# amplab/keystone

Measured on NVIDIA H100. Metric: block-LS fit samples/sec (N=1M, D=64K, k=1K), higher is better.
Workload: dtype f16x2

## Files before the change

### keystone_b200/csrc/engine.cu

```cuda
#include "engine.h"

#include <cuda_fp16.h>
#include <dlfcn.h>
#include <stdlib.h>
#include <math.h>
#include <string.h>

#include <chrono>
#include <functional>
#include <mutex>
#include <sstream>

namespace ks {

template <class F>
static void load_sym(void* lib, const char* name, F& out, const char* libname) {
  void* s = dlsym(lib, name);
  if (!s) throw KsError{KS_ERR_SOLVER, std::string("symbol ") + name + " missing from " + libname};
  out = reinterpret_cast<F>(s);
}
static void* open_first(const std::vector<const char*>& names) {
  for (const char* n : names) {
    void* h = dlopen(n, RTLD_NOW | RTLD_GLOBAL);
    if (h) return h;
// ... 493 lines not shown
  float* slab = static_cast<float*>(slab_v);
  if (src.F) {
    if (!round_out || out16 || x2) throw KsError{KS_ERR_INVALID, "unrounded / fp16 slabs only for generated features"};
    launch_center_round(src.F->d + row_begin * src.F->ld, src.F->ld, static_cast<int>(c0), shift, slab, colsum, lds, rows,
                        static_cast<int>(cols), st);
    c.launches += 1;
    return;
  }
  KmLaunch k;
  int64_t kdepth = src.d_in;
  if (x2) {
    if (!src.proj_x2 || out16 || round_out) throw KsError{KS_ERR_INVALID, "split-operand slab requested without split operands"};
    kdepth = 3 * src.d_in;
    tmap16_or_throw(&k.tmA, static_cast<const uint16_t*>(src.x3.p) + row_begin * src.ldx3, rows, kdepth, src.ldx3, 64, 128, TMAP_SW128);
    tmap16_or_throw(&k.tmB, static_cast<const uint16_t*>(src.w3.p) + c0 * src.ldw3, cols, kdepth, src.ldw3, 64, 128, TMAP_SW128);
    k.f16 = 1;
    k.p.acc_scale_ptr = src.pscale.as<float>();
  } else if (out16 && src.proj16) {
    tmap16_or_throw(&k.tmA, static_cast<const uint16_t*>(src.xop16.p) + row_begin * src.X->ld, rows, src.d_in, src.X->ld, 64, 128,
                    TMAP_SW128);
    tmap16_or_throw(&k.tmB, static_cast<const uint16_t*>(src.w16.p) + c0 * src.ldw, cols, src.d_in, src.ldw, 64, 128, TMAP_SW128);
    k.f16 = 1;
    k.p.acc_scale_ptr = src.pscale.as<float>();
  } else {
    tmap_or_throw(&k.tmA, src.xop.as<float>() + row_begin * src.X->ld, rows, src.d_in, src.X->ld, 128);
    tmap_or_throw(&k.tmB, src.Wall + c0 * src.ldw, cols, src.d_in, src.ldw, 128);
  }
  if (slab_lo && !x2) throw KsError{KS_ERR_INVALID, "a lo plane needs the split operands"};
  if (slab_lo) {
    tmap16_or_throw(&k.tmOut, slab_v, rows, cols, lds, 32, 32, TMAP_NONE);
    tmap16_or_throw(&k.tmOut2, slab_lo, rows, cols, lds, 32, 32, TMAP_NONE);
    k.out16 = 2;
  } else {
    if (out16) tmap16_or_throw(&k.tmOut, slab_v, rows, cols, lds, 32, 32, TMAP_NONE);
    else tmap_or_throw(&k.tmOut, slab, rows, cols, lds, 32);
    k.out16 = out16 ? 1 : 0;
  }
  k.p.vec0 = src.ball + c0;
  k.p.vec1 = shift;
  k.p.colsum = colsum;
  k.p.colsumsq = colsumsq;
  k.p.M = static_cast<int>(rows);
  k.p.N = static_cast<int>(cols);
  k.p.K = static_cast<int>(kdepth);
  k.p.flags = (round_out ? 0 : KM_FLAG_NO_ROUND) | (src.kind == 1 ? KM_FLAG_RECT : 0);
  k.p.rect_floor = src.rect_floor;
  k.epi = EPI_COS;
  k.num_sms = (st == c.st2) ? std::max(1, c.num_sms - c.reserve_sms) : c.num_sms;
  if (c.dyn_tiles) k.p.tile_counter = c.next_tile_counter(st);
  KS_CUDA(launch_kmajor(k, st));
  c.launches += 1;
}

const GramTile* gram_tiles(Ctx& c, int b, int kcols, bool with_g, bool with_c, int* num_tiles) {
  std::vector<int> key = {b, kcols, with_g ? 1 : 0, with_c ? 1 : 0};
  auto it = c.tile_cache.find(key);
  std::vector<GramTile> t;
  const int tm = 128, tn = 128;
  const int mb = (b + tm - 1) / tm;
  if (with_g) {
    const int nbk = (b + tn - 1) / tn;
    for (int i = 0; i < mb; ++i)
      for (int j = 0; j < nbk; ++j)
        if ((j + 1) * tn - 1 >= i * tm) t.push_back(GramTile{i, j, 0, 0});
  }
  if (with_c) {
    const int nck = (kcols + tn - 1) / tn;
    for (int i = 0; i < mb; ++i)
      for (int j = 0; j < nck; ++j) t.push_back(GramTile{i, j, 1, 0});
  }
  *num_tiles = static_cast<int>(t.size());
  if (it != c.tile_cache.end()) return it->second->as<GramTile>();
  auto buf = std::make_unique<DevBuf>();
  buf->alloc(sizeof(GramTile) * std::max<size_t>(t.size(), 1));
  KS_CUDA(cudaMemcpyAsync(buf->p, t.data(), sizeof(GramTile) * t.size(), cudaMemcpyHostToDevice, c.st));
  KS_CUDA(cudaStreamSynchronize(c.st));
  const GramTile* p = buf->as<GramTile>();
  c.tile_cache[key] = std::move(buf);
  return p;
}

void launch_gram_block(Ctx& c, const void* slab, int64_t lds, int64_t rows, int b, const void* R, int64_t ldr, int kcols,
                       float* G, int ldg, float* C, int ldc, bool with_g, bool with_c, cudaStream_t st, bool f16,
                       int64_t chunk_rows, const void* slab_lo, const void* R_lo) {
  if (rows <= 0 || b <= 0 || (!with_g && !with_c)) return;
  if (!st) st = c.st;
  const bool split = slab_lo != nullptr;
  if (split && (!f16 || (with_c && !R_lo))) throw KsError{KS_ERR_INVALID, "split Gram operands must be fp16 pairs"};
  GramLaunch g;
  int nt = 0;
  g.f16 = f16 ? 1 : 0;
  g.split = split ? 1 : 0;
  g.tiles = gram_tiles(c, b, kcols, with_g, with_c, &nt);
  g.num_tiles = nt;
  const int stage_rows = split ? 32 : f16 ? 64 : kGramStageRows;
  if (f16) {
    tmap16_or_throw(&g.tmA, slab, rows, b, lds, 64, stage_rows, TMAP_SW128);
    g.tmB0 = g.tmA;
    if (with_c) tmap16_or_throw(&g.tmB1, R, rows, kcols, ldr, 64, stage_rows, TMAP_SW128);
    else g.tmB1 = g.tmA;
    if (split) {
      tmap16_or_throw(&g.tmAlo, slab_lo, rows, b, lds, 64, stage_rows, TMAP_SW128);
      g.tmB0lo = g.tmAlo;
      if (with_c) tmap16_or_throw(&g.tmB1lo, R_lo, rows, kcols, ldr, 64, stage_rows, TMAP_SW128);
      else g.tmB1lo = g.tmAlo;
    }
  } else {
    tmap_or_throw(&g.tmA, static_cast<const float*>(slab), rows, b, lds, kGramStageRows);
    g.tmB0 = g.tmA;
    if (with_c) tmap_or_throw(&g.tmB1, static_cast<const float*>(R), rows, kcols, ldr, kGramStageRows);
    else g.tmB1 = g.tmA;
  }
  g.rows = static_cast<int>(rows);
  int64_t chunk = chunk_rows > 0 ? chunk_rows : c.gram_chunk_rows;
  if (chunk <= 0) chunk = !f16 ? 4096 : rows >= 400000 ? 16384 : rows >= 200000 ? 8192 : 4096;
  chunk = std::max<int64_t>(stage_rows, chunk / stage_rows * stage_rows);
  g.chunk_rows = static_cast<int>(chunk);
  if (with_g) tmap_or_throw(&g.tmOut0, G, b, b, ldg, 32);
  if (with_c) tmap_or_throw(&g.tmOut1, C, b, kcols, ldc, 32);
  if (!with_g) g.tmOut0 = g.tmOut1;
  if (!with_c) g.tmOut1 = g.tmOut0;
  g.n_valid0 = b;
  g.n_valid1 = kcols;
  KS_CUDA(launch_gram(g, st));
  c.launches += 1;
}

void launch_update(Ctx& c, const void* slab, int64_t lds, int64_t rows, int b, const void* bop, int64_t ldb, int k,
                   float* out, int64_t ldo, const float* cbias, int epi, bool reduce, cudaStream_t st, bool f16,
                   const float* acc_scale_ptr, const void* slab_lo, const void* bop_lo) {
  if (rows <= 0 || k <= 0 || b <= 0) return;
  if (!st) st = c.st;
  const bool split = slab_lo != nullptr;
  if (split && (!f16 || !bop_lo || epi != EPI_UPDATE)) throw KsError{KS_ERR_INVALID, "split update operands must be fp16 pairs"};
  KmLaunch u;
  u.f16 = f16 ? 1 : 0;
  u.split = split ? 1 : 0;
  u.p.acc_scale_ptr = acc_scale_ptr;
  if (split) {
    tmap16_or_throw(&u.tmA, slab, rows, b, lds, 32, 128, TMAP_SW64);
    tmap16_or_throw(&u.tmAlo, slab_lo, rows, b, lds, 32, 128, TMAP_SW64);
    tmap16_or_throw(&u.tmB, bop, k, b, ldb, 32, 128, TMAP_SW64);
    tmap16_or_throw(&u.tmBlo, bop_lo, k, b, ldb, 32, 128, TMAP_SW64);
  } else if (f16) {
    tmap16_or_throw(&u.tmA, slab, rows, b, lds, 64, 128, TMAP_SW128);
    tmap16_or_throw(&u.tmB, bop, k, b, ldb, 64, 128, TMAP_SW128);
  } else {
// ... 2152 lines not shown
```

### keystone_b200/csrc/engine.h

```cpp
#pragma once
#include <cuda_runtime.h>
#include <cusolverDn.h>
#include <nccl.h>
#include <stdint.h>

#include <map>
#include <memory>
#include <string>
#include <unordered_map>
#include <vector>

#include "../../include/keystone_b200.h"
#include "kernels.h"

namespace ks {

struct KsError {
  int code;
  std::string msg;
};

#define KS_CUDA(call)                                                                                   \
  do {                                                                                                  \
    cudaError_t e__ = (call);                                                                           \
// ... 238 lines not shown
  int64_t add(std::unique_ptr<Matrix> m);
  int64_t add(std::unique_ptr<Model> m);
  cudaEvent_t get_event();
  void span_begin(int phase, cudaStream_t s = nullptr);
  void span_end(cudaStream_t s = nullptr);
  void collect_spans(double out_ms[PH_COUNT]);
  void allreduce_f32(float* p, size_t n, bool prep = false);
  void allreduce_f64(double* p, size_t n, bool prep = false);
  void allreduce_on(void* p, size_t n, bool f64, ncclComm_t cm, cudaStream_t s);
  DevBuf tile_counters;
  int tile_counter_next = 0;
  int dyn_tiles = 1;
  int* next_tile_counter(cudaStream_t s);
  std::vector<cudaEvent_t> fit_events;
  void allreduce_max_u32(unsigned* p, size_t n);
  void ensure_solver();
  void potrf(double* H, int n, int info_slot, cudaStream_t s);
  void potrs(const double* H, int n, double* B, int nrhs, int info_slot, cudaStream_t s);
  void check_infos(int used_slots);
  void check_async(const char* what);
};

struct FeatMap {
  float* Wall = nullptr;
  float* Wfull = nullptr;
  int kind = 0;
  float rect_floor = 0.f;
  float* ball = nullptr;
  int64_t ldw = 0, d_in = 0;
  int64_t D = 0;
};
struct FeatSrc : FeatMap {
  Matrix* F = nullptr;
  Matrix* X = nullptr;
  DevBuf xop;
  DevBuf xop16, w16, pscale;
  bool proj16 = false;
  DevBuf x3, w3;
  int64_t ldx3 = 0, ldw3 = 0;
  bool proj_x2 = false;
  DevBuf wcat, wcat_full, bcat;
  int64_t n_rows = 0;
  DevBuf zeros;
};
void make_feat_src(Ctx& c, int64_t features, int64_t x_in, const int64_t* rfs, int32_t n_rfs, FeatSrc& out,
                   int precision = 0);
void prepare_generated_operands(Ctx& c, FeatSrc& out, int precision);
void derive_feat_src(Ctx& c, const FeatSrc& src, Matrix* X, FeatSrc& out, int precision);
void produce_slab(Ctx& c, FeatSrc& src, int64_t c0, int64_t cols, const float* shift, void* slab, int64_t lds,
                  int64_t row_begin, int64_t rows, bool round_out = true, float* colsum = nullptr, cudaStream_t st = nullptr,
                  bool out16 = false, bool x2 = false,
                  void* slab_lo = nullptr,
                  double* colsumsq = nullptr);
const GramTile* gram_tiles(Ctx& c, int b, int kcols, bool with_g, bool with_c, int* num_tiles);
void launch_gram_block(Ctx& c, const void* slab, int64_t lds, int64_t rows, int b, const void* R, int64_t ldr, int kcols,
                       float* G, int ldg, float* C, int ldc, bool with_g, bool with_c, cudaStream_t st = nullptr,
                       bool f16 = false, int64_t chunk_rows = 0,
                       const void* slab_lo = nullptr, const void* R_lo = nullptr);
void launch_update(Ctx& c, const void* slab, int64_t lds, int64_t rows, int b, const void* bop, int64_t ldb, int k,
                   float* out, int64_t ldo, const float* cbias, int epi, bool reduce, cudaStream_t st = nullptr,
                   bool f16 = false, const float* acc_scale_ptr = nullptr,
                   const void* slab_lo = nullptr, const void* bop_lo = nullptr);

int64_t fit_bwls(Ctx& c, FeatSrc& src, Matrix& Y, int bs, int num_iter, double lam, double w, int64_t nf_opt,
                 int precision = KS_PRECISION_TF32);
void launch_set_f64(double* p, double v, cudaStream_t st);
void launch_scale_f64(const double* src, double scale, float* dst, double* dst64, int n, cudaStream_t st);
int64_t fit_lbfgs(Ctx& c, FeatSrc& src, Matrix& Y, bool fit_intercept, int num_corrections, double convergence_tol, int num_iterations,
                  double reg_param, int precision);
void model_alloc_host(Model& m);
void model_block_to_host(Model& m, int j, cudaStream_t s);
void model_intercept_to_host(Model& m, cudaStream_t s);

std::unique_ptr<Matrix> new_matrix(int64_t rows, int64_t cols);
int64_t gaussian_kernel_create(Ctx& c, Matrix& X, double gamma);
std::unique_ptr<Matrix> gaussian_kernel_block(Ctx& c, const GaussKernel& K, Matrix& x, int64_t col0, int64_t cols);
int64_t fit_krr(Ctx& c, const std::shared_ptr<GaussKernel>& K, Matrix& Y, double lam, int bs, int epochs,
                const int32_t* order_or_null);
std::unique_ptr<Matrix> kernel_model_apply(Ctx& c, Model& md, Matrix& x);
int64_t kernel_model_from_host(Ctx& c, const std::shared_ptr<GaussKernel>& K, const double* const* xs, const int64_t* block_rows,
                               int32_t n_blocks, int64_t k, int32_t block_size);

int64_t fit_pca(Ctx& c, Matrix& X, int dims);
int64_t fit_zca(Ctx& c, Matrix& X, double eps);
int64_t approx_range(Ctx& c, Matrix& X, const double* omega_colmajor, int l, int q);
int64_t fit_approx_pca(Ctx& c, Matrix& X, const double* omega_colmajor, int dims, int q, int p);
void debug_gram_f64(Ctx& c, Matrix& A, Matrix* B, const double* shift_a, const double* shift_b, double* out, int64_t ld_out);
struct GramOperand {
  const float* f32 = nullptr;
  const double* f64 = nullptr;
  int64_t ld = 0;
  int cols = 0;
  const double* shift = nullptr;
};
void gram_f64(Ctx& c, const GramOperand& a, const GramOperand* b, int64_t rows, double* out, int64_t ldo, double* flops = nullptr);
void skinny_f64(Ctx& c, const GramOperand& a, int64_t rows, const double* B, int64_t ldb, int l, double* Y, int64_t ldy);

std::unique_ptr<Matrix> lcs_extract(Ctx& c, Matrix& images, int x_dim, int y_dim, int channels, int stride, int stride_start,
                                    int sub_patch_size);
int64_t gmm_create(Ctx& c, const double* means_colmajor, const double* vars_colmajor, const double* weights, int64_t dim, int64_t k,
                   double weight_threshold);
std::unique_ptr<Matrix> gmm_posteriors(Ctx& c, const Gmm& g, Matrix& X);
std::unique_ptr<Matrix> fisher_vector_apply(Ctx& c, const Gmm& g, Matrix& X, const int64_t* item_offsets, int64_t n_items);
std::unique_ptr<Matrix> normalize_rows(Ctx& c, Matrix& in);
void launch_signed_sqrt(Ctx& c, const float* in, float* out, int64_t n);
void launch_gmm_estep(Ctx& c, const Gmm& g, const Matrix& X, int64_t row0, int64_t rows, double* Q, float* out, int64_t ldo, int epi,
                      double* row_out);
// ... 71 lines not shown
```

### keystone_b200/csrc/kernels.h

```cpp
#pragma once
#include <cuda.h>
#include <cuda_runtime.h>
#include <stdint.h>

namespace ks {

static constexpr int kGramStageRows = 32;
static constexpr int kPadCols = 32;

enum { EPI_COS = 0, EPI_UPDATE = 1, EPI_APPLY = 2, EPI_POOL = 3, EPI_RBF = 4 };

struct GramTile {
  int m_blk;
  int n_blk;
  int which;
  int pad;
};
struct GramLaunch {
  CUtensorMap tmA, tmB0, tmB1;
  CUtensorMap tmOut0, tmOut1;
  CUtensorMap tmAlo, tmB0lo, tmB1lo;
  const GramTile* tiles;
  int num_tiles;
  int rows;
  int chunk_rows;
  int n_valid0, n_valid1;
  int f16 = 0;
  int split = 0;
};
enum { KM_FLAG_NO_ROUND = 1, KM_FLAG_REDUCE = 2, KM_FLAG_RECT = 8 };
struct KmParams {
  const float* vec0;
  float rect_floor = 0.f;
  const float* vec1;
  float* colsum;
  float acc_scale = 1.f;
  const float* acc_scale_ptr = nullptr;
  const unsigned* pool_mask = nullptr;
  union {
    float* pool_out = nullptr;
    double* colsumsq;
  };
  int64_t pool_out_ld = 0;
  int patches_per_image = 0, n_pools = 0;
  float pool_alpha = 0.f;
  int* tile_counter = nullptr;
  const float* row_vec = nullptr;
  float gamma = 0.f;
  int M, N, K;
  int flags;
};
struct KmLaunch {
  CUtensorMap tmA, tmB;
  CUtensorMap tmOut;
  CUtensorMap tmOut2;
  CUtensorMap tmAlo, tmBlo;
  KmParams p;
  int epi;
  int num_sms;
  int f16 = 0;
  int split = 0;
  int out16 = 0;
};

int make_tmap_2d(CUtensorMap* out, const float* base, int64_t rows, int64_t cols, int64_t ld, int box_rows);
enum { TMAP_SW128 = 0, TMAP_SW64 = 1, TMAP_NONE = 2 };
int make_tmap_any(CUtensorMap* out, const void* base, int64_t rows, int64_t cols, int64_t ld, int box_cols, int box_rows,
                  int elem_bytes, int swizzle);
cudaError_t launch_gram(const GramLaunch& g, cudaStream_t st);
cudaError_t launch_kmajor(const KmLaunch& k, cudaStream_t st);
unsigned int read_wait_timeout_flag();
cudaError_t launch_chol_solve(const double* L, const double* Dinv, int n, double* B, int k, cudaStream_t st);
cudaError_t launch_tri_inv_tiles(const double* L, int n, double* Dinv, cudaStream_t st);
size_t chol_solve_dinv_doubles(int n);

void launch_f32_repitch_rows(const float* src, int64_t src_ld, float* dst, int64_t dst_ld, int64_t rows, int64_t cols,
// ... 54 lines not shown
```

### keystone_b200/csrc/tc_common.cuh

```cuda
#pragma once
#include <cuda.h>
#include <cuda_fp16.h>
#include <cuda_runtime.h>
#include <stdint.h>

namespace ks {

__device__ unsigned int g_wait_timeout_flag = 0;

static constexpr unsigned long long kWaitBudgetCycles = 6000000000ull;

__device__ __forceinline__ uint32_t smem_u32(const void* p) {
  return static_cast<uint32_t>(__cvta_generic_to_shared(p));
}

__device__ __forceinline__ bool elect_one() {
  uint32_t pred = 0;
  asm volatile(
      "{\n\t"
      ".reg .pred P;\n\t"
      "elect.sync _|P, 0xffffffff;\n\t"
      "selp.u32 %0, 1, 0, P;\n\t"
      "}\n"
      : "=r"(pred));
  return pred != 0;
}

__device__ __forceinline__ void named_bar_sync(int id, int count) {
  asm volatile("bar.sync %0, %1;" ::"r"(id), "r"(count) : "memory");
}

__device__ __forceinline__ void mbar_init(uint64_t* bar, uint32_t count) {
  asm volatile("mbarrier.init.shared::cta.b64 [%0], %1;" ::"r"(smem_u32(bar)), "r"(count));
}
__device__ __forceinline__ void fence_barrier_init() {
  asm volatile("fence.mbarrier_init.release.cluster;" ::: "memory");
}
__device__ __forceinline__ void fence_proxy_async() {
  asm volatile("fence.proxy.async.shared::cta;" ::: "memory");
}
__device__ __forceinline__ void mbar_arrive_expect_tx(uint64_t* bar, uint32_t bytes) {
  asm volatile("mbarrier.arrive.expect_tx.shared::cta.b64 _, [%0], %1;" ::"r"(smem_u32(bar)), "r"(bytes)
               : "memory");
}
__device__ __forceinline__ void mbar_arrive(uint64_t* bar) {
  asm volatile("mbarrier.arrive.shared::cta.b64 _, [%0];" ::"r"(smem_u32(bar)) : "memory");
}
__device__ __forceinline__ bool mbar_try_wait(uint64_t* bar, uint32_t parity) {
  uint32_t ok;
  asm volatile(
      "{\n\t"
      ".reg .pred P;\n\t"
      "mbarrier.try_wait.parity.shared::cta.b64 P, [%1], %2;\n\t"
      "selp.u32 %0, 1, 0, P;\n\t"
      "}\n"
      : "=r"(ok)
      : "r"(smem_u32(bar)), "r"(parity)
      : "memory");
  return ok != 0;
}
__device__ __forceinline__ void mbar_wait(uint64_t* bar, uint32_t parity) {
  if (mbar_try_wait(bar, parity)) return;
  const unsigned long long t0 = clock64();
  while (!mbar_try_wait(bar, parity)) {
    if (clock64() - t0 > kWaitBudgetCycles) {
      atomicExch(&g_wait_timeout_flag, 1u + (blockIdx.x << 8) + (threadIdx.x >> 5));
      __trap();
    }
  }
}

__device__ __forceinline__ void tma_prefetch_desc(const CUtensorMap* m) {
  asm volatile("prefetch.tensormap [%0];" ::"l"(reinterpret_cast<uint64_t>(m)) : "memory");
}
__device__ __forceinline__ void tma_load_2d(void* smem_dst, const CUtensorMap* m, uint64_t* bar, int32_t c0,
                                            int32_t c1) {
  asm volatile(
      "cp.async.bulk.tensor.2d.shared::cluster.global.mbarrier::complete_tx::bytes [%0], [%1, {%3, %4}], [%2];"
      ::"r"(smem_u32(smem_dst)), "l"(reinterpret_cast<uint64_t>(m)), "r"(smem_u32(bar)), "r"(c0), "r"(c1)
      : "memory");
}

__device__ __forceinline__ void tma_store_2d(const CUtensorMap* m, const void* smem_src, int32_t c0, int32_t c1) {
  asm volatile("cp.async.bulk.tensor.2d.global.shared::cta.bulk_group [%0, {%2, %3}], [%1];" ::"l"(
                   reinterpret_cast<uint64_t>(m)),
               "r"(smem_u32(smem_src)), "r"(c0), "r"(c1)
               : "memory");
}
__device__ __forceinline__ void tma_reduce_add_2d(const CUtensorMap* m, const void* smem_src, int32_t c0, int32_t c1) {
  asm volatile("cp.reduce.async.bulk.tensor.2d.global.shared::cta.add.bulk_group [%0, {%2, %3}], [%1];" ::"l"(
                   reinterpret_cast<uint64_t>(m)),
               "r"(smem_u32(smem_src)), "r"(c0), "r"(c1)
               : "memory");
}
__device__ __forceinline__ void bulk_commit() { asm volatile("cp.async.bulk.commit_group;" ::: "memory"); }
__device__ __forceinline__ void bulk_wait_read0() { asm volatile("cp.async.bulk.wait_group.read 0;" ::: "memory"); }
__device__ __forceinline__ void bulk_wait0() { asm volatile("cp.async.bulk.wait_group 0;" ::: "memory"); }
__device__ __forceinline__ void bulk_wait_read1() { asm volatile("cp.async.bulk.wait_group.read 1;" ::: "memory"); }

__device__ __forceinline__ void stage_row_sw128(uint8_t* buf, int lane, const float (&o)[32]) {
  uint8_t* row = buf + lane * 128;
#pragma unroll
  for (int c = 0; c < 8; ++c)
    *reinterpret_cast<float4*>(row + ((c ^ (lane & 7)) << 4)) = make_float4(o[4 * c], o[4 * c + 1], o[4 * c + 2], o[4 * c + 3]);
}

template <int SW = 1>
__device__ __forceinline__ uint64_t make_wgmma_desc(uint32_t saddr, uint32_t lbo_bytes, uint32_t sbo_bytes) {
  uint64_t d = 0;
  d |= static_cast<uint64_t>((saddr & 0x3FFFF) >> 4);
  d |= static_cast<uint64_t>((lbo_bytes >> 4) & 0x3FFF) << 16;
  d |= static_cast<uint64_t>((sbo_bytes >> 4) & 0x3FFF) << 32;
  d |= static_cast<uint64_t>(SW) << 62;
  return d;
}

template <int N>
__device__ __forceinline__ void setmaxnreg_dec() { asm volatile("setmaxnreg.dec.sync.aligned.u32 %0;" ::"n"(N) : "memory"); }
template <int N>
__device__ __forceinline__ void setmaxnreg_inc() { asm volatile("setmaxnreg.inc.sync.aligned.u32 %0;" ::"n"(N) : "memory"); }

__device__ __forceinline__ void wgmma_fence() { asm volatile("wgmma.fence.sync.aligned;" ::: "memory"); }
__device__ __forceinline__ void wgmma_commit() { asm volatile("wgmma.commit_group.sync.aligned;" ::: "memory"); }
template <int N>
__device__ __forceinline__ void wgmma_wait() { asm volatile("wgmma.wait_group.sync.aligned %0;" ::"n"(N) : "memory"); }
__device__ __forceinline__ void wgmma_fence_acc(float (&d)[64]) {
#pragma unroll
  for (int i = 0; i < 64; ++i) asm volatile("" : "+f"(d[i])::"memory");
}

#define KS_WG_D64                                                                                                          \
  "{%0, %1, %2, %3, %4, %5, %6, %7, %8, %9, %10, %11, %12, %13, %14, %15, %16, %17, %18, %19, %20, %21, %22, %23, %24, %25, " \
// ... 46 lines not shown
```

### keystone_b200/csrc/tc_kernels.cu

```cuda
#include <type_traits>

#include "tc_common.cuh"
#include "kernels.h"

namespace ks {

static constexpr int kThreads = 384;
static constexpr int kTileM = 128, kTileN = 128;
static constexpr int kStages = 4;
static constexpr int kRawLd = 65;
static constexpr int kRawBytes = 2 * 64 * kRawLd * 4;
static constexpr int kStagingBytes = 8 * 4096;
static constexpr int kVecBytes = 8 * 64 * 4;
static constexpr int kEpiBytes = kStagingBytes + kRawBytes + kVecBytes;
static constexpr int kStageBytes = 32768;
static constexpr int kSmemBytes = kStages * kStageBytes + kEpiBytes + 1024  + 256 ;
static_assert(kSmemBytes <= 227 * 1024, "shared memory per block");

struct SmemLayout {
  uint8_t* stages;
  uint8_t* staging;
  float* raw;
  float* vec;
  uint64_t* full_bar;
// ... 67 lines not shown
__device__ __forceinline__ void sts_f32(uint32_t addr, float v) { asm volatile("st.shared.f32 [%0], %1;" ::"r"(addr), "f"(v)); }
__device__ __forceinline__ float lds_f32(uint32_t addr) {
  float v;
  asm volatile("ld.shared.f32 %0, [%1];" : "=f"(v) : "r"(addr));
  return v;
}
__device__ __forceinline__ void wgmma_acc_to_tile(const float (&acc)[64], uint32_t tile, int g, int w, int lane) {
  const uint32_t base = tile + 4 * ((64 * g + 16 * w + (lane >> 2)) * kTileLd + 2 * (lane & 3));
#pragma unroll
  for (int j = 0; j < 16; ++j)
#pragma unroll
    for (int e = 0; e < 4; ++e) sts_f32(base + 4 * ((8 * (e >> 1)) * kTileLd + 8 * j + (e & 1)), acc[4 * j + e]);
}

template <typename ToRaw, typename Chunk>
__device__ __forceinline__ void epilogue_slabs(float* raw, int g, int w, int lane, ToRaw to_raw, Chunk chunk) {
#pragma unroll
  for (int slab = 0; slab < kTileN / 64; ++slab) {
    to_raw(raw, slab);
    named_bar_sync(1 + g, 128);
    float o[32];
    const float* src = raw + (32 * (w & 1) + lane) * kRawLd + 32 * (w >> 1);
#pragma unroll
    for (int i = 0; i < 32; ++i) o[i] = src[i];
    named_bar_sync(1 + g, 128);
    chunk(o, slab, 32 * (w & 1), slab * 64 + 32 * (w >> 1));
  }
}

template <bool F16, bool SPLIT = false>
struct GramCfg {
  static constexpr int PLANES = SPLIT ? 4 : 2;
  static constexpr int SR = SPLIT ? 32 : F16 ? 64 : 32;
  static constexpr int CW = F16 ? 64 : 32;
  static constexpr int NBOX = kTileM / CW;
  static constexpr int BOX_BYTES = SR * 128;
  static constexpr int A_BYTES = NBOX * BOX_BYTES;
  static_assert(PLANES * A_BYTES == kStageBytes, "stage size");
  static_assert(!SPLIT || F16, "split operands are fp16 pairs");
};

template <int BOX_BYTES>
__device__ __forceinline__ uint32_t ld_mn_tf32(const uint8_t* tile, int c, int r) {
  return *reinterpret_cast<const uint32_t*>(tile + (c >> 5) * BOX_BYTES + r * 128 + (((((c & 31) >> 2) ^ (r & 7))) << 4) +
                                            ((c & 3) << 2));
}

template <bool F16, bool SPLIT>
__global__ void __launch_bounds__(kThreads, 1)
gram_tn_kernel(const __grid_constant__ CUtensorMap tmA, const __grid_constant__ CUtensorMap tmB0,
               const __grid_constant__ CUtensorMap tmB1, const __grid_constant__ CUtensorMap tmOut0,
               const __grid_constant__ CUtensorMap tmOut1, const __grid_constant__ CUtensorMap tmAlo,
               const __grid_constant__ CUtensorMap tmB0lo, const __grid_constant__ CUtensorMap tmB1lo,
               const GramTile* __restrict__ tiles, int num_tiles, int rows, int chunk_rows, int n_valid0, int n_valid1) {
  using Cfg = GramCfg<F16, SPLIT>;
  constexpr int SR = Cfg::SR;
  extern __shared__ uint8_t smem_raw[];
  const SmemLayout L = carve_smem(smem_raw);

  const int warp = threadIdx.x >> 5;
  const int lane = threadIdx.x & 31;
  const int wg = warp >> 2;
  const GramTile tile = tiles[blockIdx.x % num_tiles];
  const int chunk = blockIdx.x / num_tiles;
  const int row0 = chunk * chunk_rows;
  const int nrows = min(chunk_rows, rows - row0);
  const int ksteps = (nrows + SR - 1) / SR;
  const int m0 = tile.m_blk * kTileM;
  const int n0 = tile.n_blk * kTileN;
  const CUtensorMap* tmB = tile.which ? &tmB1 : &tmB0;
  const CUtensorMap* tmBlo = tile.which ? &tmB1lo : &tmB0lo;
  const CUtensorMap* tmOut = tile.which ? &tmOut1 : &tmOut0;

  if (threadIdx.x == 0) {
    tma_prefetch_desc(&tmA);
    tma_prefetch_desc(tmB);
    if (SPLIT) {
      tma_prefetch_desc(&tmAlo);
      tma_prefetch_desc(tmBlo);
    }
    tma_prefetch_desc(tmOut);
    for (int s = 0; s < kStages; ++s) {
      mbar_init(&L.full_bar[s], 1);
      mbar_init(&L.empty_bar[s], 8);
    }
    fence_barrier_init();
  }
  __syncthreads();

  if (wg == 0) {
    if (SPLIT) setmaxnreg_dec<40>();
    if (warp == 0 && elect_one()) {
      for (int ks = 0; ks < ksteps; ++ks) {
        const int s = ks % kStages;
        const uint32_t ph = (ks / kStages) & 1;
        mbar_wait(&L.empty_bar[s], ph ^ 1);
        mbar_arrive_expect_tx(&L.full_bar[s], kStageBytes);
        uint8_t* sA = L.stages + s * kStageBytes;
        const int r = row0 + ks * SR;
        const CUtensorMap* maps[4] = {&tmA, SPLIT ? &tmAlo : tmB, tmB, tmBlo};
#pragma unroll
        for (int pl = 0; pl < Cfg::PLANES; ++pl) {
          const int c0 = (pl < Cfg::PLANES / 2) ? m0 : n0;
#pragma unroll
          for (int i = 0; i < Cfg::NBOX; ++i)
            tma_load_2d(sA + pl * Cfg::A_BYTES + i * Cfg::BOX_BYTES, maps[pl], &L.full_bar[s], c0 + Cfg::CW * i, r);
        }
      }
    }
    return;
  }
  if (SPLIT) setmaxnreg_inc<232>();

  const int g = wg - 1;
  const int w = warp & 3;
  float acc[64];
#pragma unroll
  for (int i = 0; i < 64; ++i) acc[i] = 0.f;

  if (SPLIT) {
    float acc_x[64];
#pragma unroll
    for (int i = 0; i < 64; ++i) acc_x[i] = 0.f;
    wgmma_fence_acc(acc);
    wgmma_fence_acc(acc_x);
    int prev = -1;
    for (int ks = 0; ks < ksteps; ++ks) {
      const int s = ks % kStages;
      mbar_wait(&L.full_bar[s], (ks / kStages) & 1);
      const uint32_t st = smem_u32(L.stages + s * kStageBytes);
      const uint32_t sAhi = st + g * Cfg::BOX_BYTES, sAlo = sAhi + Cfg::A_BYTES;
      const uint32_t sBhi = st + 2 * Cfg::A_BYTES, sBlo = st + 3 * Cfg::A_BYTES;
      wgmma_fence();
#pragma unroll
      for (int kk = 0; kk < SR / 16; ++kk)
        wgmma_f16_n128<1, 1>(acc, make_wgmma_desc(sAhi + kk * 2048, Cfg::BOX_BYTES, 1024),
                             make_wgmma_desc(sBhi + kk * 2048, Cfg::BOX_BYTES, 1024), 1);
#pragma unroll
      for (int kk = 0; kk < SR / 16; ++kk) {
        wgmma_f16_n128<1, 1>(acc_x, make_wgmma_desc(sAlo + kk * 2048, Cfg::BOX_BYTES, 1024),
                             make_wgmma_desc(sBhi + kk * 2048, Cfg::BOX_BYTES, 1024), 1);
        wgmma_f16_n128<1, 1>(acc_x, make_wgmma_desc(sAhi + kk * 2048, Cfg::BOX_BYTES, 1024),
                             make_wgmma_desc(sBlo + kk * 2048, Cfg::BOX_BYTES, 1024), 1);
      }
      wgmma_commit();
      if (prev >= 0) {
        wgmma_wait<1>();
        if (lane == 0) mbar_arrive(&L.empty_bar[prev]);
      }
      prev = s;
    }
    wgmma_wait<0>();
    wgmma_fence_acc(acc);
    wgmma_fence_acc(acc_x);
#pragma unroll
    for (int i = 0; i < 64; ++i) acc[i] = __fadd_rn(acc[i], acc_x[i]);
  } else if (F16) {
    wgmma_fence_acc(acc);
    int prev = -1;
    for (int ks = 0; ks < ksteps; ++ks) {
      const int s = ks % kStages;
      mbar_wait(&L.full_bar[s], (ks / kStages) & 1);
      const uint32_t sA = smem_u32(L.stages + s * kStageBytes) + g * Cfg::BOX_BYTES;
      const uint32_t sB = smem_u32(L.stages + s * kStageBytes) + Cfg::A_BYTES;
      wgmma_fence();
#pragma unroll
      for (int kk = 0; kk < SR / 16; ++kk) {
        const uint64_t ad = make_wgmma_desc(sA + kk * 2048, Cfg::BOX_BYTES, 1024);
        const uint64_t bd = make_wgmma_desc(sB + kk * 2048, Cfg::BOX_BYTES, 1024);
        wgmma_f16_n128<1, 1>(acc, ad, bd, 1);
      }
      wgmma_commit();
      if (prev >= 0) {
        wgmma_wait<1>();
        if (lane == 0) mbar_arrive(&L.empty_bar[prev]);
      }
      prev = s;
    }
    wgmma_wait<0>();
    wgmma_fence_acc(acc);
  } else {
    const int mrow = 64 * g + 32 * (w & 1);
    const int ncol = 64 * (w >> 1);
    const int gq = lane >> 2, tq = lane & 3;
    for (int ks = 0; ks < ksteps; ++ks) {
      const int s = ks % kStages;
      mbar_wait(&L.full_bar[s], (ks / kStages) & 1);
      const uint8_t* sA = L.stages + s * kStageBytes;
      const uint8_t* sB = sA + Cfg::A_BYTES;
#pragma unroll
      for (int k = 0; k < SR; k += 8) {
        uint32_t a[2][4], b[8][2];
#pragma unroll
        for (int mi = 0; mi < 2; ++mi) {
          const int m = mrow + 16 * mi + gq;
          a[mi][0] = ld_mn_tf32<Cfg::BOX_BYTES>(sA, m, k + tq);
          a[mi][1] = ld_mn_tf32<Cfg::BOX_BYTES>(sA, m + 8, k + tq);
          a[mi][2] = ld_mn_tf32<Cfg::BOX_BYTES>(sA, m, k + tq + 4);
          a[mi][3] = ld_mn_tf32<Cfg::BOX_BYTES>(sA, m + 8, k + tq + 4);
        }
#pragma unroll
        for (int ni = 0; ni < 8; ++ni) {
          const int n = ncol + 8 * ni + gq;
          b[ni][0] = ld_mn_tf32<Cfg::BOX_BYTES>(sB, n, k + tq);
          b[ni][1] = ld_mn_tf32<Cfg::BOX_BYTES>(sB, n, k + tq + 4);
        }
#pragma unroll
        for (int mi = 0; mi < 2; ++mi)
#pragma unroll
          for (int ni = 0; ni < 8; ++ni) mma_tf32_16x8x8(&acc[(mi * 8 + ni) * 4], a[mi], b[ni]);
      }
      __syncwarp();
      if (lane == 0) mbar_arrive(&L.empty_bar[s]);
    }
  }

  const int n_valid = tile.which ? n_valid1 : n_valid0;
  uint8_t* buf = L.staging + (warp - 4) * 4096;
  float* raw = L.raw + g * 64 * kRawLd;
  auto to_raw = [&](float* rw, int slab) {
    if (F16) {
      wgmma_acc_to_raw(acc, rw, slab, w, lane);
    } else if ((w >> 1) == slab) {
#pragma unroll
      for (int mi = 0; mi < 2; ++mi)
#pragma unroll
        for (int ni = 0; ni < 8; ++ni)
#pragma unroll
          for (int e = 0; e < 4; ++e)
            rw[(32 * (w & 1) + 16 * mi + (lane >> 2) + 8 * (e >> 1)) * kRawLd + 8 * ni + 2 * (lane & 3) + (e & 1)] =
                acc[(mi * 8 + ni) * 4 + e];
    }
  };
  auto chunk_fn = [&](float (&o)[32], int, int r_off, int c_off) {
    const int col = n0 + c_off;
    if (col >= n_valid) return;
    if (lane == 0) bulk_wait_read0();
    __syncwarp();
    stage_row_sw128(buf, lane, o);
    fence_proxy_async();
    __syncwarp();
    if (lane == 0) {
      tma_reduce_add_2d(tmOut, buf, col, m0 + 64 * g + r_off);
      bulk_commit();
    }
  };
  epilogue_slabs(raw, g, w, lane, to_raw, chunk_fn);
  if (lane == 0) bulk_wait0();
}

__device__ __forceinline__ float cos_reduced(float x) {
  const float kInv2Pi = 0.15915494309189535f;
  const float k2PiHi = 6.2831854820251465f;
  const float k2PiLo = -1.7484555314695172e-7f;
  const float kMagic = 12582912.0f;
  const float k = __fadd_rn(__fmaf_rn(x, kInv2Pi, kMagic), -kMagic);
  float r = fmaf(-k, k2PiHi, x);
  r = fmaf(-k, k2PiLo, r);
  return __cosf(r);
}

__device__ __forceinline__ void stage_row_f16(uint8_t* buf, int lane, const float (&o)[32]) {
  uint4* row = reinterpret_cast<uint4*>(buf + lane * 64);
#pragma unroll
  for (int c = 0; c < 4; ++c) {
    __half2 h0 = __floats2half2_rn(o[8 * c + 0], o[8 * c + 1]);
    __half2 h1 = __floats2half2_rn(o[8 * c + 2], o[8 * c + 3]);
    __half2 h2 = __floats2half2_rn(o[8 * c + 4], o[8 * c + 5]);
    __half2 h3 = __floats2half2_rn(o[8 * c + 6], o[8 * c + 7]);
    uint4 v;
    v.x = *reinterpret_cast<uint32_t*>(&h0);
    v.y = *reinterpret_cast<uint32_t*>(&h1);
    v.z = *reinterpret_cast<uint32_t*>(&h2);
    v.w = *reinterpret_cast<uint32_t*>(&h3);
    row[c] = v;
  }
}

__device__ __forceinline__ void stage_row_f16x2(uint8_t* buf, int lane, const float (&o)[32]) {
  uint4* row_hi = reinterpret_cast<uint4*>(buf + lane * 64);
  uint4* row_lo = reinterpret_cast<uint4*>(buf + 2048 + lane * 64);
#pragma unroll
  for (int c = 0; c < 4; ++c) {
    uint32_t wh[4], wl[4];
#pragma unroll
    for (int e = 0; e < 4; ++e) {
      const float a = o[8 * c + 2 * e], b = o[8 * c + 2 * e + 1];
      const __half2 h = __floats2half2_rn(a, b);
      const float2 hf = __half22float2(h);
      const __half2 l = __floats2half2_rn(a - hf.x, b - hf.y);
      wh[e] = *reinterpret_cast<const uint32_t*>(&h);
      wl[e] = *reinterpret_cast<const uint32_t*>(&l);
    }
    row_hi[c] = make_uint4(wh[0], wh[1], wh[2], wh[3]);
    row_lo[c] = make_uint4(wl[0], wl[1], wl[2], wl[3]);
  }
}

template <int EPI, int OUT16>
__device__ __forceinline__ void km_chunk(const KmParams& p, const CUtensorMap* tmOut, const CUtensorMap* tmOut2, const float (&a)[32],
                                         const float* vs, uint8_t* sbuf, int slot, int row0, int col0, int lane, float ascale) {
// ... 362 lines not shown
    epilogue_slabs(raw, g, w, lane, to_raw, chunk_fn);
  }
  if (lane == 0) bulk_wait0();
}

typedef CUresult (*PFN_encodeTiled)(CUtensorMap*, CUtensorMapDataType, cuuint32_t, void*, const cuuint64_t*,
                                    const cuuint64_t*, const cuuint32_t*, const cuuint32_t*, CUtensorMapInterleave,
                                    CUtensorMapSwizzle, CUtensorMapL2promotion, CUtensorMapFloatOOBfill);

static PFN_encodeTiled get_encode_fn() {
  static PFN_encodeTiled fn = nullptr;
  if (!fn) {
    void* p = nullptr;
    cudaDriverEntryPointQueryResult qres;
    if (cudaGetDriverEntryPoint("cuTensorMapEncodeTiled", &p, cudaEnableDefault, &qres) != cudaSuccess ||
        qres != cudaDriverEntryPointSuccess)
      return nullptr;
    fn = reinterpret_cast<PFN_encodeTiled>(p);
  }
  return fn;
}

int make_tmap_2d(CUtensorMap* out, const float* base, int64_t rows, int64_t cols, int64_t ld, int box_rows) {
  return make_tmap_any(out, base, rows, cols, ld, 32, box_rows, 4, TMAP_SW128);
}

int make_tmap_any(CUtensorMap* out, const void* base, int64_t rows, int64_t cols, int64_t ld, int box_cols, int box_rows,
                  int elem_bytes, int swizzle) {
  PFN_encodeTiled fn = get_encode_fn();
  if (!fn) return -1;
  cuuint64_t dims[2] = {static_cast<cuuint64_t>(cols), static_cast<cuuint64_t>(rows)};
  cuuint64_t strides[1] = {static_cast<cuuint64_t>(ld) * static_cast<cuuint64_t>(elem_bytes)};
  cuuint32_t box[2] = {static_cast<cuuint32_t>(box_cols), static_cast<cuuint32_t>(box_rows)};
  cuuint32_t estr[2] = {1u, 1u};
  const CUtensorMapSwizzle sw = swizzle == TMAP_SW128  ? CU_TENSOR_MAP_SWIZZLE_128B
                                : swizzle == TMAP_SW64 ? CU_TENSOR_MAP_SWIZZLE_64B
                                                       : CU_TENSOR_MAP_SWIZZLE_NONE;
  CUresult r = fn(out, elem_bytes == 2 ? CU_TENSOR_MAP_DATA_TYPE_FLOAT16 : CU_TENSOR_MAP_DATA_TYPE_FLOAT32, 2,
                  const_cast<void*>(base), dims, strides, box, estr, CU_TENSOR_MAP_INTERLEAVE_NONE, sw,
                  CU_TENSOR_MAP_L2_PROMOTION_L2_256B, CU_TENSOR_MAP_FLOAT_OOB_FILL_NONE);
  return r == CUDA_SUCCESS ? 0 : -static_cast<int>(r) - 1000;
}

template <typename K>
static cudaError_t set_smem_attr_once(K kern, bool& done, int bytes = kSmemBytes) {
  if (!done) {
    cudaError_t e = cudaFuncSetAttribute(kern, cudaFuncAttributeMaxDynamicSharedMemorySize, bytes);
    if (e != cudaSuccess) return e;
    done = true;
  }
  return cudaSuccess;
}

template <bool F16, bool SPLIT>
static cudaError_t launch_gram_t(const GramLaunch& g, cudaStream_t st) {
  if (g.chunk_rows % GramCfg<F16, SPLIT>::SR != 0) return cudaErrorInvalidValue;
  auto kern = gram_tn_kernel<F16, SPLIT>;
  static bool attr_done = false;
  cudaError_t e = set_smem_attr_once(kern, attr_done);
  if (e != cudaSuccess) return e;
  const int chunks = (g.rows + g.chunk_rows - 1) / g.chunk_rows;
  const unsigned grid = static_cast<unsigned>(chunks) * static_cast<unsigned>(g.num_tiles);
  if (grid == 0) return cudaSuccess;
  kern<<<grid, kThreads, kSmemBytes, st>>>(g.tmA, g.tmB0, g.tmB1, g.tmOut0, g.tmOut1, SPLIT ? g.tmAlo : g.tmA, SPLIT ? g.tmB0lo : g.tmB0,
                                           SPLIT ? g.tmB1lo : g.tmB1, g.tiles, g.num_tiles, g.rows, g.chunk_rows, g.n_valid0, g.n_valid1);
  return cudaGetLastError();
}

cudaError_t launch_gram(const GramLaunch& g, cudaStream_t st) {
  if (g.split) return g.f16 ? launch_gram_t<true, true>(g, st) : cudaErrorInvalidValue;
  return g.f16 ? launch_gram_t<true, false>(g, st) : launch_gram_t<false, false>(g, st);
}

template <int EPI, bool F16, int OUT16, bool SPLIT = false>
static cudaError_t launch_km_t(const KmLaunch& k, cudaStream_t st) {
  auto kern = gemm_kmajor_kernel<EPI, F16, OUT16, SPLIT>;
  static bool attr_done = false;
  cudaError_t e = set_smem_attr_once(kern, attr_done, km_smem_bytes(EPI));
  if (e != cudaSuccess) return e;
  const int m_tiles = (k.p.M + kTileM - 1) / kTileM;
  const int n_tiles = (k.p.N + kTileN - 1) / kTileN;
  const long long total = static_cast<long long>(m_tiles) * n_tiles;
  if (total == 0) return cudaSuccess;
  const unsigned grid = static_cast<unsigned>(total < k.num_sms ? total : k.num_sms);
  kern<<<grid, km_threads(EPI), km_smem_bytes(EPI), st>>>(k.tmA, k.tmB, k.tmOut, OUT16 == 2 ? k.tmOut2 : k.tmOut, SPLIT ? k.tmAlo : k.tmA,
                                           SPLIT ? k.tmBlo : k.tmB, k.p);
  return cudaGetLastError();
}

cudaError_t launch_kmajor(const KmLaunch& k, cudaStream_t st) {
  if (k.split) return (k.f16 && k.epi == EPI_UPDATE) ? launch_km_t<EPI_UPDATE, true, 0, true>(k, st) : cudaErrorInvalidValue;
  if (k.epi == EPI_POOL) return k.f16 ? launch_km_t<EPI_POOL, true, 0>(k, st) : cudaErrorInvalidValue;
  if (k.epi == EPI_RBF) return (k.f16 && k.out16 == 2) ? launch_km_t<EPI_RBF, true, 2>(k, st) : cudaErrorInvalidValue;
  if (k.f16 && k.epi == EPI_APPLY) return launch_km_t<EPI_APPLY, true, 0>(k, st);
  if (k.f16 && k.epi == EPI_UPDATE) return launch_km_t<EPI_UPDATE, true, 0>(k, st);
  if (k.out16 == 2 && k.epi == EPI_COS) return k.f16 ? launch_km_t<EPI_COS, true, 2>(k, st) : cudaErrorInvalidValue;
  if (k.out16 && k.f16 && k.epi == EPI_COS) return launch_km_t<EPI_COS, true, 1>(k, st);
  if (k.f16 && k.epi == EPI_COS) return launch_km_t<EPI_COS, true, 0>(k, st);
  if (k.out16 && k.epi == EPI_COS) return launch_km_t<EPI_COS, false, 1>(k, st);
  switch (k.epi) {
    case EPI_COS: return launch_km_t<EPI_COS, false, 0>(k, st);
    case EPI_UPDATE: return launch_km_t<EPI_UPDATE, false, 0>(k, st);
    case EPI_APPLY: return launch_km_t<EPI_APPLY, false, 0>(k, st);
    default: return cudaErrorInvalidValue;
  }
}

unsigned int read_wait_timeout_flag() {
  unsigned int v = 0;
  cudaMemcpyFromSymbol(&v, g_wait_timeout_flag, sizeof(v));
  return v;
}

}
```

Before: 298,400.

## Pair Gram tiles into 2-CTA clusters sharing operands via TMA multicast

Gram tiles are grouped into pairs that share either the A row-block or the B column-block. Each pair launches as a 2-CTA cluster, and each CTA multicasts half of the shared operand into both CTAs' shared memory. Empty barriers now need arrivals from both CTAs before a stage is reused. The goal is to roughly halve global/L2 traffic for the shared operand. In exchange it adds cluster synchronisation, cross-CTA barrier coupling, and wasted idle CTAs for unpaired solo tiles. The split path is unchanged apart from the pair indexing.

Result: no change. 297,900, median of 6 (-0.1%).

```diff
diff --git a/keystone_b200/csrc/engine.cu b/keystone_b200/csrc/engine.cu
--- a/keystone_b200/csrc/engine.cu
+++ b/keystone_b200/csrc/engine.cu
@@ -569,24 +569,41 @@
   c.launches += 1;
 }
 
-const GramTile* gram_tiles(Ctx& c, int b, int kcols, bool with_g, bool with_c, int* num_tiles) {
+const GramTile* gram_tiles(Ctx& c, int b, int kcols, bool with_g, bool with_c, int* num_pairs) {
   std::vector<int> key = {b, kcols, with_g ? 1 : 0, with_c ? 1 : 0};
   auto it = c.tile_cache.find(key);
   std::vector<GramTile> t;
   const int tm = 128, tn = 128;
   const int mb = (b + tm - 1) / tm;
-  if (with_g) {
-    const int nbk = (b + tn - 1) / tn;
-    for (int i = 0; i < mb; ++i)
-      for (int j = 0; j < nbk; ++j)
-        if ((j + 1) * tn - 1 >= i * tm) t.push_back(GramTile{i, j, 0, 0});
-  }
-  if (with_c) {
-    const int nck = (kcols + tn - 1) / tn;
-    for (int i = 0; i < mb; ++i)
-      for (int j = 0; j < nck; ++j) t.push_back(GramTile{i, j, 1, 0});
-  }
-  *num_tiles = static_cast<int>(t.size());
+  auto add_pairs = [&](int which, int ncb, bool upper) {
+    std::vector<std::vector<int>> left(ncb);
+    for (int i = 0; i < mb; ++i) {
+      std::vector<int> js;
+      for (int j = 0; j < ncb; ++j)
+        if (!upper || (j + 1) * tn - 1 >= i * tm) js.push_back(j);
+      size_t q = 0;
+      for (; q + 1 < js.size(); q += 2) {
+        t.push_back(GramTile{i, js[q], which, GRAM_SHARE_A});
+        t.push_back(GramTile{i, js[q + 1], which, GRAM_SHARE_A});
+      }
+      if (q < js.size()) left[js[q]].push_back(i);
+    }
+    for (int j = 0; j < ncb; ++j) {
+      const std::vector<int>& is = left[j];
+      size_t q = 0;
+      for (; q + 1 < is.size(); q += 2) {
+        t.push_back(GramTile{is[q], j, which, GRAM_SHARE_B});
+        t.push_back(GramTile{is[q + 1], j, which, GRAM_SHARE_B});
+      }
+      if (q < is.size()) {
+        t.push_back(GramTile{is[q], j, which, GRAM_SOLO});
+        t.push_back(GramTile{is[q], j, which, GRAM_SOLO});
+      }
+    }
+  };
+  if (with_g) add_pairs(0, (b + tn - 1) / tn, true);
+  if (with_c) add_pairs(1, (kcols + tn - 1) / tn, false);
+  *num_pairs = static_cast<int>(t.size() / 2);
   if (it != c.tile_cache.end()) return it->second->as<GramTile>();
   auto buf = std::make_unique<DevBuf>();
   buf->alloc(sizeof(GramTile) * std::max<size_t>(t.size(), 1));
@@ -609,7 +626,7 @@
   g.f16 = f16 ? 1 : 0;
   g.split = split ? 1 : 0;
   g.tiles = gram_tiles(c, b, kcols, with_g, with_c, &nt);
-  g.num_tiles = nt;
+  g.num_pairs = nt;
   const int stage_rows = split ? 32 : f16 ? 64 : kGramStageRows;
   if (f16) {
     tmap16_or_throw(&g.tmA, slab, rows, b, lds, 64, stage_rows, TMAP_SW128);
diff --git a/keystone_b200/csrc/engine.h b/keystone_b200/csrc/engine.h
--- a/keystone_b200/csrc/engine.h
+++ b/keystone_b200/csrc/engine.h
@@ -314,7 +314,7 @@
                   bool out16 = false, bool x2 = false,
                   void* slab_lo = nullptr,
                   double* colsumsq = nullptr);
-const GramTile* gram_tiles(Ctx& c, int b, int kcols, bool with_g, bool with_c, int* num_tiles);
+const GramTile* gram_tiles(Ctx& c, int b, int kcols, bool with_g, bool with_c, int* num_pairs);
 void launch_gram_block(Ctx& c, const void* slab, int64_t lds, int64_t rows, int b, const void* R, int64_t ldr, int kcols,
                        float* G, int ldg, float* C, int ldc, bool with_g, bool with_c, cudaStream_t st = nullptr,
                        bool f16 = false, int64_t chunk_rows = 0,
diff --git a/keystone_b200/csrc/kernels.h b/keystone_b200/csrc/kernels.h
--- a/keystone_b200/csrc/kernels.h
+++ b/keystone_b200/csrc/kernels.h
@@ -10,18 +10,19 @@
 
 enum { EPI_COS = 0, EPI_UPDATE = 1, EPI_APPLY = 2, EPI_POOL = 3, EPI_RBF = 4 };
 
+enum { GRAM_SHARE_A = 0, GRAM_SHARE_B = 1, GRAM_SOLO = 2 };
 struct GramTile {
   int m_blk;
   int n_blk;
   int which;
-  int pad;
+  int share;
 };
 struct GramLaunch {
   CUtensorMap tmA, tmB0, tmB1;
   CUtensorMap tmOut0, tmOut1;
   CUtensorMap tmAlo, tmB0lo, tmB1lo;
   const GramTile* tiles;
-  int num_tiles;
+  int num_pairs;
   int rows;
   int chunk_rows;
   int n_valid0, n_valid1;
diff --git a/keystone_b200/csrc/tc_common.cuh b/keystone_b200/csrc/tc_common.cuh
--- a/keystone_b200/csrc/tc_common.cuh
+++ b/keystone_b200/csrc/tc_common.cuh
@@ -70,6 +70,20 @@
   }
 }
 
+__device__ __forceinline__ uint32_t cluster_ctarank() {
+  uint32_t r;
+  asm volatile("mov.u32 %0, %%cluster_ctarank;" : "=r"(r));
+  return r;
+}
+__device__ __forceinline__ void cluster_sync() {
+  asm volatile("barrier.cluster.arrive.relaxed;\n\tbarrier.cluster.wait;" ::: "memory");
+}
+__device__ __forceinline__ void mbar_arrive_remote(uint64_t* bar, uint32_t rank) {
+  uint32_t remote;
+  asm volatile("mapa.shared::cluster.u32 %0, %1, %2;" : "=r"(remote) : "r"(smem_u32(bar)), "r"(rank));
+  asm volatile("mbarrier.arrive.shared::cluster.b64 _, [%0];" ::"r"(remote) : "memory");
+}
+
 __device__ __forceinline__ void tma_prefetch_desc(const CUtensorMap* m) {
   asm volatile("prefetch.tensormap [%0];" ::"l"(reinterpret_cast<uint64_t>(m)) : "memory");
 }
@@ -78,6 +92,15 @@
   asm volatile(
       "cp.async.bulk.tensor.2d.shared::cluster.global.mbarrier::complete_tx::bytes [%0], [%1, {%3, %4}], [%2];"
       ::"r"(smem_u32(smem_dst)), "l"(reinterpret_cast<uint64_t>(m)), "r"(smem_u32(bar)), "r"(c0), "r"(c1)
+      : "memory");
+}
+
+__device__ __forceinline__ void tma_load_2d_multicast(void* smem_dst, const CUtensorMap* m, uint64_t* bar, int32_t c0, int32_t c1,
+                                                      uint16_t cta_mask) {
+  asm volatile(
+      "cp.async.bulk.tensor.2d.shared::cluster.global.mbarrier::complete_tx::bytes.multicast::cluster [%0], [%1, {%4, %5}], [%2], "
+      "%3;" ::"r"(smem_u32(smem_dst)),
+      "l"(reinterpret_cast<uint64_t>(m)), "r"(smem_u32(bar)), "h"(cta_mask), "r"(c0), "r"(c1)
       : "memory");
 }
 
diff --git a/keystone_b200/csrc/tc_kernels.cu b/keystone_b200/csrc/tc_kernels.cu
--- a/keystone_b200/csrc/tc_kernels.cu
+++ b/keystone_b200/csrc/tc_kernels.cu
@@ -143,7 +143,7 @@
                const __grid_constant__ CUtensorMap tmB1, const __grid_constant__ CUtensorMap tmOut0,
                const __grid_constant__ CUtensorMap tmOut1, const __grid_constant__ CUtensorMap tmAlo,
                const __grid_constant__ CUtensorMap tmB0lo, const __grid_constant__ CUtensorMap tmB1lo,
-               const GramTile* __restrict__ tiles, int num_tiles, int rows, int chunk_rows, int n_valid0, int n_valid1) {
+               const GramTile* __restrict__ tiles, int num_pairs, int rows, int chunk_rows, int n_valid0, int n_valid1) {
   using Cfg = GramCfg<F16, SPLIT>;
   constexpr int SR = Cfg::SR;
   extern __shared__ uint8_t smem_raw[];
@@ -152,8 +152,12 @@
   const int warp = threadIdx.x >> 5;
   const int lane = threadIdx.x & 31;
   const int wg = warp >> 2;
-  const GramTile tile = tiles[blockIdx.x % num_tiles];
-  const int chunk = blockIdx.x / num_tiles;
+  constexpr bool CLUSTER = !SPLIT;
+  const uint32_t rank = CLUSTER ? cluster_ctarank() : (blockIdx.x & 1);
+  const int pair = (blockIdx.x >> 1) % num_pairs;
+  const int chunk = (blockIdx.x >> 1) / num_pairs;
+  const GramTile tile = tiles[2 * pair + rank];
+  const bool paired = CLUSTER && tile.share != GRAM_SOLO;
   const int row0 = chunk * chunk_rows;
   const int nrows = min(chunk_rows, rows - row0);
   const int ksteps = (nrows + SR - 1) / SR;
@@ -173,15 +177,28 @@
     tma_prefetch_desc(tmOut);
     for (int s = 0; s < kStages; ++s) {
       mbar_init(&L.full_bar[s], 1);
-      mbar_init(&L.empty_bar[s], 8);
+      mbar_init(&L.empty_bar[s], paired ? 16 : 8);
     }
     fence_barrier_init();
   }
-  __syncthreads();
+  if (CLUSTER) cluster_sync();
+  else __syncthreads();
+  if (tile.share == GRAM_SOLO && rank != 0) {
+    if (CLUSTER) cluster_sync();
+    return;
+  }
+  auto release = [&](int s) {
+    if (lane == 0) {
+      mbar_arrive(&L.empty_bar[s]);
+      if (paired) mbar_arrive_remote(&L.empty_bar[s], rank ^ 1u);
+    }
+  };
 
   if (wg == 0) {
     if (SPLIT) setmaxnreg_dec<40>();
     if (warp == 0 && elect_one()) {
+      constexpr int HALF = Cfg::PLANES / 2 * Cfg::NBOX / 2;
+      const bool share_a = tile.share == GRAM_SHARE_A;
       for (int ks = 0; ks < ksteps; ++ks) {
         const int s = ks % kStages;
         const uint32_t ph = (ks / kStages) & 1;
@@ -192,13 +209,21 @@
         const CUtensorMap* maps[4] = {&tmA, SPLIT ? &tmAlo : tmB, tmB, tmBlo};
 #pragma unroll
         for (int pl = 0; pl < Cfg::PLANES; ++pl) {
-          const int c0 = (pl < Cfg::PLANES / 2) ? m0 : n0;
-#pragma unroll
-          for (int i = 0; i < Cfg::NBOX; ++i)
-            tma_load_2d(sA + pl * Cfg::A_BYTES + i * Cfg::BOX_BYTES, maps[pl], &L.full_bar[s], c0 + Cfg::CW * i, r);
-        }
-      }
-    }
+          const bool a_side = pl < Cfg::PLANES / 2;
+          const int c0 = a_side ? m0 : n0;
+          const bool shared = paired && a_side == share_a;
+#pragma unroll
+          for (int i = 0; i < Cfg::NBOX; ++i) {
+            uint8_t* dst = sA + pl * Cfg::A_BYTES + i * Cfg::BOX_BYTES;
+            if (!shared)
+              tma_load_2d(dst, maps[pl], &L.full_bar[s], c0 + Cfg::CW * i, r);
+            else if (((pl % (Cfg::PLANES / 2)) * Cfg::NBOX + i) / HALF == static_cast<int>(rank))
+              tma_load_2d_multicast(dst, maps[pl], &L.full_bar[s], c0 + Cfg::CW * i, r, 0x3);
+          }
+        }
+      }
+    }
+    if (CLUSTER) cluster_sync();
     return;
   }
   if (SPLIT) setmaxnreg_inc<232>();
@@ -237,7 +262,7 @@
       wgmma_commit();
       if (prev >= 0) {
         wgmma_wait<1>();
-        if (lane == 0) mbar_arrive(&L.empty_bar[prev]);
+        release(prev);
       }
       prev = s;
     }
@@ -264,7 +289,7 @@
       wgmma_commit();
       if (prev >= 0) {
         wgmma_wait<1>();
-        if (lane == 0) mbar_arrive(&L.empty_bar[prev]);
+        release(prev);
       }
       prev = s;
     }
@@ -302,7 +327,7 @@
           for (int ni = 0; ni < 8; ++ni) mma_tf32_16x8x8(&acc[(mi * 8 + ni) * 4], a[mi], b[ni]);
       }
       __syncwarp();
-      if (lane == 0) mbar_arrive(&L.empty_bar[s]);
+      release(s);
     }
   }
 
@@ -338,6 +363,7 @@
   };
   epilogue_slabs(raw, g, w, lane, to_raw, chunk_fn);
   if (lane == 0) bulk_wait0();
+  if (CLUSTER) cluster_sync();
 }
 
 __device__ __forceinline__ float cos_reduced(float x) {
@@ -806,6 +832,23 @@
   return cudaSuccess;
 }
 
+template <typename... P, typename... Args>
+static cudaError_t launch_cluster2(void (*kern)(P...), unsigned grid, int threads, int smem, cudaStream_t st, Args&&... args) {
+  cudaLaunchConfig_t cfg = {};
+  cfg.gridDim = dim3(grid);
+  cfg.blockDim = dim3(threads);
+  cfg.dynamicSmemBytes = static_cast<size_t>(smem);
+  cfg.stream = st;
+  cudaLaunchAttribute attr[1];
+  attr[0].id = cudaLaunchAttributeClusterDimension;
+  attr[0].val.clusterDim.x = 2;
+  attr[0].val.clusterDim.y = 1;
+  attr[0].val.clusterDim.z = 1;
+  cfg.attrs = attr;
+  cfg.numAttrs = 1;
+  return cudaLaunchKernelEx(&cfg, kern, std::forward<Args>(args)...);
+}
+
 template <bool F16, bool SPLIT>
 static cudaError_t launch_gram_t(const GramLaunch& g, cudaStream_t st) {
   if (g.chunk_rows % GramCfg<F16, SPLIT>::SR != 0) return cudaErrorInvalidValue;
@@ -814,11 +857,16 @@
   cudaError_t e = set_smem_attr_once(kern, attr_done);
   if (e != cudaSuccess) return e;
   const int chunks = (g.rows + g.chunk_rows - 1) / g.chunk_rows;
-  const unsigned grid = static_cast<unsigned>(chunks) * static_cast<unsigned>(g.num_tiles);
+  const unsigned grid = 2u * static_cast<unsigned>(chunks) * static_cast<unsigned>(g.num_pairs);
   if (grid == 0) return cudaSuccess;
-  kern<<<grid, kThreads, kSmemBytes, st>>>(g.tmA, g.tmB0, g.tmB1, g.tmOut0, g.tmOut1, SPLIT ? g.tmAlo : g.tmA, SPLIT ? g.tmB0lo : g.tmB0,
-                                           SPLIT ? g.tmB1lo : g.tmB1, g.tiles, g.num_tiles, g.rows, g.chunk_rows, g.n_valid0, g.n_valid1);
-  return cudaGetLastError();
+  if (SPLIT) {
+    kern<<<grid, kThreads, kSmemBytes, st>>>(g.tmA, g.tmB0, g.tmB1, g.tmOut0, g.tmOut1, g.tmAlo, g.tmB0lo, g.tmB1lo, g.tiles, g.num_pairs,
+                                             g.rows, g.chunk_rows, g.n_valid0, g.n_valid1);
+    return cudaGetLastError();
+  }
+  return launch_cluster2(kern, grid, kThreads, kSmemBytes, st, g.tmA, g.tmB0, g.tmB1, g.tmOut0, g.tmOut1, SPLIT ? g.tmAlo : g.tmA,
+                         SPLIT ? g.tmB0lo : g.tmB0, SPLIT ? g.tmB1lo : g.tmB1, g.tiles, g.num_pairs, g.rows, g.chunk_rows,
+                         g.n_valid0, g.n_valid1);
 }
 
 cudaError_t launch_gram(const GramLaunch& g, cudaStream_t st) {
```
